# gkaissis/PriMIA

Measured on AMD Instinct MI355X. Metric: images_per_sec, higher is better.
Workload: dtype bf16; 1 GPU; ResNet-18 federated-client training step (fwd+loss+bwd+SGD), batch 256/client, 3x224x224, 1 client per GPU; batch_per_client=256, clients=1, sync_every_n_batch=3, dp_sgd=False

## Files before the change

### primia_amd/build.py

```python
import concurrent.futures
import os
import shutil
import subprocess
import sys

HERE = os.path.dirname(os.path.abspath(__file__))
CSRC = os.path.join(HERE, "csrc")
OBJ = os.path.join(CSRC, "_build")
ISA = os.path.join(OBJ, "isa")
LIB = os.path.join(HERE, "libprimia_hip.so")
ARCH = "gfx950"
FLAGS = ["-O3", "-std=c++17", "-fPIC", f"--offload-arch={ARCH}", "-Wno-unused-result"]


def source_digest(files=None):
    import hashlib

    names = sorted(f for f in os.listdir(CSRC) if f.endswith((".hip", ".h"))) if files is None else sorted(files)
    paths = [os.path.join(CSRC, f) for f in names]
    if files is None:
        paths.append(os.path.join(HERE, "..", "include", "primia_hip.h"))
    h = hashlib.sha256()
    for q in paths:
        h.update(os.path.basename(q).encode() + b"\0")
        import re

        text = re.sub(r"/\*.*?\*/", "", open(q, "r", encoding="utf-8", errors="replace").read(), flags=re.S)
        for line in text.splitlines():
            code = line.split("//", 1)[0].rstrip()
            if code:
                h.update(code.encode() + b"\n")
    return h.hexdigest()


def _hipcc():
    for c in ("/opt/rocm/bin/hipcc", "hipcc"):
        if os.path.isabs(c) and os.path.exists(c):
            return c
    return "hipcc"


def _newer(src, dst, deps=()):
    if not os.path.exists(dst):
        return True
    t = os.path.getmtime(dst)
    return any(os.path.getmtime(p) > t for p in (src, *deps))


def build(force=False, verbose=True):
    os.makedirs(OBJ, exist_ok=True)
    headers = [os.path.join(CSRC, f) for f in os.listdir(CSRC) if f.endswith(".h")]
    headers.append(os.path.join(HERE, "..", "include", "primia_hip.h"))
    sources = sorted(f for f in os.listdir(CSRC) if f.endswith(".hip"))
    jobs = []
    for f in sources:
        src = os.path.join(CSRC, f)
        obj = os.path.join(OBJ, f[:-4] + ".o")
        if force or _newer(src, obj, headers) or not os.path.exists(os.path.join(ISA, f[:-4] + ".s")):
            jobs.append((src, obj))

    def compile_one(job):
        src, obj = job
        name = os.path.basename(src)[:-4]
        tmp = os.path.join(OBJ, "tmp_" + name)
        shutil.rmtree(tmp, ignore_errors=True)
        os.makedirs(tmp)
        cmd = [_hipcc(), *FLAGS, "-save-temps=obj", "-c", src, "-o", os.path.join(tmp, name + ".o")]
        r = subprocess.run(cmd, capture_output=True, text=True)
        if r.returncode == 0:
            os.makedirs(ISA, exist_ok=True)
            os.replace(os.path.join(tmp, f"{name}-hip-amdgcn-amd-amdhsa-{ARCH}.s"), os.path.join(ISA, name + ".s"))
            os.replace(os.path.join(tmp, name + ".o"), obj)
        shutil.rmtree(tmp, ignore_errors=True)
        return src, r.returncode, r.stdout + r.stderr

    if jobs:
        with concurrent.futures.ThreadPoolExecutor(max_workers=min(6, len(jobs))) as ex:
            for src, rc, out in ex.map(compile_one, jobs):
                if verbose:
                    print(f"[primia build] {os.path.basename(src)}: {'ok' if rc == 0 else 'FAILED'}")
                if rc != 0:
                    raise RuntimeError(f"hipcc failed for {src}:\n{out}")
    objs = [os.path.join(OBJ, f[:-4] + ".o") for f in sources]
    if jobs or force or not os.path.exists(LIB):
        cmd = [_hipcc(), "-shared", "-fPIC", f"--offload-arch={ARCH}", "-o", LIB, *objs]
        r = subprocess.run(cmd, capture_output=True, text=True)
        if r.returncode != 0:
            raise RuntimeError("link failed:\n" + r.stdout + r.stderr)
        if verbose:
            print(f"[primia build] linked {LIB}")
    return LIB


PROBE_LIB = os.path.join(HERE, "..", "tools", "micro", "libprimia_probe.so")
PROBE_SOURCES = ("conv3x3_c64.hip", "conv_s2lh.hip", "options.hip")


def build_probe(extra_flags=()):
    build(verbose=False)
    objs = []
    for f in sorted(x for x in os.listdir(CSRC) if x.endswith(".hip")):
        if f in PROBE_SOURCES:
            os.makedirs(os.path.join(OBJ, "probe"), exist_ok=True)
            obj = os.path.join(OBJ, "probe", f[:-4] + ".o")
            cmd = [_hipcc(), *FLAGS, "-DPRIMIA_PROBE=1", *extra_flags, "-c", os.path.join(CSRC, f), "-o", obj]
            r = subprocess.run(cmd, capture_output=True, text=True)
            if r.returncode != 0:
                raise RuntimeError(f"hipcc failed for {f} (probe):\n{r.stdout}{r.stderr}")
        else:
            obj = os.path.join(OBJ, f[:-4] + ".o")
        objs.append(obj)
    r = subprocess.run([_hipcc(), "-shared", "-fPIC", f"--offload-arch={ARCH}", "-o", PROBE_LIB, *objs],
                       capture_output=True, text=True)
    if r.returncode != 0:
        raise RuntimeError("link failed:\n" + r.stdout + r.stderr)
    print(f"[primia build] linked {os.path.normpath(PROBE_LIB)}")
    return PROBE_LIB


if __name__ == "__main__":
    if "--probe" in sys.argv:
        build_probe()
    else:
        build(force="--force" in sys.argv)
```

### primia_amd/csrc/options.h

```cpp
#pragma once

namespace primia {

#define PRIMIA_OPTIONS(X)                                                                                              \
    X(lh2, 1)                                        \
    X(lh2_bm, 0)                                      \
    X(lh4, 1)                \
    X(c64_blocks, 512)                                         \
    X(c64_dbg, 0)                      \
    X(c64_stages, 4)                                                      \
    X(s2lh, 1)               \
    X(s2lh_dbg, 0)

enum OptId : int {
#define PRIMIA_OPT_ENUM(name, def) kOpt_##name,
    PRIMIA_OPTIONS(PRIMIA_OPT_ENUM)
#undef PRIMIA_OPT_ENUM
        kOptCount
};

extern int g_options[kOptCount];

inline int opt(OptId id) { return __atomic_load_n(&g_options[id], __ATOMIC_RELAXED); }

}

#define PRIMIA_OPT(name) (::primia::opt(::primia::kOpt_##name))
```

### primia_amd/csrc/options.hip

```cpp
#include <string.h>

#include <atomic>

#include "common.h"
#include "options.h"

#ifndef PRIMIA_PROBE
#define PRIMIA_PROBE 0
#endif

namespace primia {

int g_options[kOptCount] = {
#define PRIMIA_OPT_DEF(name, def) def,
    PRIMIA_OPTIONS(PRIMIA_OPT_DEF)
#undef PRIMIA_OPT_DEF
};

static const char* const kOptNames[kOptCount] = {
#define PRIMIA_OPT_NAME(name, def) #name,
    PRIMIA_OPTIONS(PRIMIA_OPT_NAME)
#undef PRIMIA_OPT_NAME
};

static const int kOptDefaults[kOptCount] = {
#define PRIMIA_OPT_DEF(name, def) def,
    PRIMIA_OPTIONS(PRIMIA_OPT_DEF)
#undef PRIMIA_OPT_DEF
};

static std::atomic<int64_t> g_options_epoch{0};

static int find_option(const char* name) {
    if (!name) return -1;
    for (int i = 0; i < kOptCount; ++i)
        if (!strcmp(name, kOptNames[i])) return i;
    return -1;
}

}

using namespace primia;

extern "C" {

int primia_set_option(const char* name, int value) {
    const int i = find_option(name);
    if (i < 0) return PRIMIA_ERR_ARG;
#if !PRIMIA_PROBE
    if ((i == kOpt_c64_dbg || i == kOpt_s2lh_dbg) && value != 0) return PRIMIA_ERR_UNSUPPORTED;
#endif
    if (__atomic_exchange_n(&g_options[i], value, __ATOMIC_RELAXED) != value)
        g_options_epoch.fetch_add(1, std::memory_order_release);
    return PRIMIA_OK;
}

int64_t primia_options_epoch(void) { return g_options_epoch.load(std::memory_order_acquire); }

int primia_get_option(const char* name, int* value) {
    const int i = find_option(name);
    if (i < 0 || !value) return PRIMIA_ERR_ARG;
    *value = __atomic_load_n(&g_options[i], __ATOMIC_RELAXED);
    return PRIMIA_OK;
}

int primia_reset_options(void) {
    bool moved = false;
    for (int i = 0; i < kOptCount; ++i) moved |= __atomic_exchange_n(&g_options[i], kOptDefaults[i], __ATOMIC_RELAXED) != kOptDefaults[i];
    if (moved) g_options_epoch.fetch_add(1, std::memory_order_release);
    return PRIMIA_OK;
}

int primia_option_count(void) { return kOptCount; }

int primia_option_name(int index, char* buf, int buf_len) {
    if (index < 0 || index >= kOptCount || !buf || buf_len <= (int)strlen(kOptNames[index])) return PRIMIA_ERR_ARG;
    strcpy(buf, kOptNames[index]);
    return PRIMIA_OK;
}

}
```

### primia_amd/csrc/stem_bwd_fused.hip

```cpp
#include <stdlib.h>

#include "conv_wgrad.h"

namespace primia {

__device__ __attribute__((aligned(16))) const unsigned char kStemFusedZeroPage[16] = {0};

__device__ __forceinline__ void sbf_dma16(const void* g, unsigned lds_addr) {
    asm volatile("s_mov_b32 m0, %1\n\ts_nop 0\n\tglobal_load_lds_dwordx4 %0, off" ::"v"(g), "s"(lds_addr) : "memory");
}

typedef int sbf_i32x4 __attribute__((ext_vector_type(4)));

__device__ __forceinline__ void sbf_bdma16(unsigned voff, sbf_i32x4 rsrc, unsigned lds_addr) {
    asm volatile("s_mov_b32 m0, %2\n\ts_nop 0\n\tbuffer_load_dwordx4 %0, %1, 0 offen lds"
                 ::"v"(voff), "s"(rsrc), "s"(lds_addr) : "memory");
}

__device__ __forceinline__ sbf_i32x4 sbf_rsrc(const void* base, long bytes) {
    const unsigned long long a = (unsigned long long)base;
    sbf_i32x4 r;
    r[0] = (int)(unsigned)a;
    r[1] = (int)(unsigned)(a >> 32) & 0xffff;
    r[2] = (int)(unsigned)(bytes > 0xfffffff0L ? 0xfffffff0L : bytes);
    r[3] = 0x00020000;
#pragma unroll
    for (int j = 0; j < 4; ++j) r[j] = __builtin_amdgcn_readfirstlane(r[j]);
    return r;
}
constexpr unsigned kSbfOob = 0xfffffff0u;

__device__ __forceinline__ int sbf_key(int slot) { return ((slot >> 1) & 1) | (((slot >> 3) & 1) << 1); }

__device__ __forceinline__ void sbf_wait_vmcnt(int n) {
    switch (n) {
        case 0: asm volatile("s_waitcnt vmcnt(0)" ::: "memory"); break;
        case 1: asm volatile("s_waitcnt vmcnt(1)" ::: "memory"); break;
        case 2: asm volatile("s_waitcnt vmcnt(2)" ::: "memory"); break;
        case 3: asm volatile("s_waitcnt vmcnt(3)" ::: "memory"); break;
        case 4: asm volatile("s_waitcnt vmcnt(4)" ::: "memory"); break;
        case 5: asm volatile("s_waitcnt vmcnt(5)" ::: "memory"); break;
        case 6: asm volatile("s_waitcnt vmcnt(6)" ::: "memory"); break;
        case 7: asm volatile("s_waitcnt vmcnt(7)" ::: "memory"); break;
        default: asm volatile("s_waitcnt vmcnt(8)" ::: "memory"); break;
    }
}

struct StemFusedParams {
    const bf16* xp;
    const bf16* y;
    const bf16* dpool;
    const uint8_t* argmax;
    const float *gamma, *beta, *mean, *invstd, *dbeta, *dgamma;
    float inv_m;
    float* dw;
    float* ws;
    int N, Hp, Wp, Ho, Wo, Hq, Wq;
    int PH, PW, PPI;
    int total, per_block;
    int debug;
};

constexpr int kSbfXB = 7 * 1024;
constexpr int kSbfTile = 16 * 1024;
constexpr int kSbfRaw = kSbfTile + 9 * 1024;
constexpr int kSbfRing = 5;
constexpr int kSbfRaw0 = 3 * kSbfXB;
constexpr int kSbfLds = kSbfRaw0 + kSbfRing * kSbfRaw;

__global__ __launch_bounds__(1024) void stem_bwd_fused_kernel(StemFusedParams p) {
    typedef __attribute__((address_space(3))) bf16x4_t* lds4_t;
    extern __shared__ __attribute__((aligned(16))) char smem[];
    const int tid = threadIdx.x, lane = tid & 63;
    const int wave = __builtin_amdgcn_readfirstlane(tid >> 6);
    const unsigned lds0 = (unsigned)(size_t)(__attribute__((address_space(3))) char*)smem;

    const int t0 = blockIdx.x * p.per_block;
    int t1 = t0 + p.per_block;
    if (t1 > p.total) t1 = p.total;
    const int n = t1 - t0;
    if (n <= 0) return;
    int cn = t0 / p.PPI, cph, cpw;
    {
        const int rem = t0 - cn * p.PPI;
        cph = rem / p.PW;
        cpw = rem - cph * p.PW;
    }
    auto advance = [&](int& an, int& aph, int& apw) {
        if (++apw == p.PW) {
            apw = 0;
            if (++aph == p.PH) {
                aph = 0;
                ++an;
            }
        }
    };

    if (wave >= 8) {
        const int tw = wave - 8;
        const int npc = tw == 0 ? 4 : 3;
        const sbf_i32x4 rs_y = sbf_rsrc(p.y, (long)p.N * p.Ho * p.Wo * 128);
        const sbf_i32x4 rs_g = sbf_rsrc(p.dpool, (long)p.N * p.Hq * p.Wq * 128);
        const sbf_i32x4 rs_c = sbf_rsrc(p.argmax, (long)p.N * p.Hq * p.Wq * 64);
        unsigned prel[4];
        int prow[4], pcol[4];
#pragma unroll
        for (int it = 0; it < 4; ++it) {
            const int idx = tw + 8 * it;
            prow[it] = pcol[it] = 0;
            if (idx < 16) {
                const int slot = idx * 8 + (lane >> 3), sl = lane & 7;
                const int chunk = ((((sl >> 1) ^ sbf_key(slot)) << 1) | (sl & 1));
                prel[it] = (unsigned)((((slot >> 4) * p.Wo + (slot & 15)) * 64 + chunk * 8) * 2);
            } else {
                const bool grad = idx < 22;
                const int G = (grad ? idx - 16 : idx - 22) * 64 + lane;
                const int slot = grad ? G >> 3 : G >> 2, sub = grad ? G & 7 : G & 3;
                const int row = slot / 9, col = slot - 9 * row;
                prow[it] = slot < 45 ? row : 1 << 20;
                pcol[it] = col;
                prel[it] = (unsigned)(grad ? (row * p.Wq + col) * 128 + sub * 16 : (row * p.Wq + col) * 64 + sub * 16);
            }
        }
        auto stage_raw = [&](int rbuf) {
            const unsigned ybase = (unsigned)(((cn * p.Ho + cph * 8) * p.Wo + cpw * 16) * 128);
            const int A0 = cph * 4, B0 = cpw * 8;
            const unsigned wpix = (unsigned)((cn * p.Hq + A0) * p.Wq + B0);
            const int rmax = p.Hq - A0, cmax = p.Wq - B0;
            advance(cn, cph, cpw);
#pragma unroll
            for (int it = 0; it < 4; ++it) {
                const int idx = tw + 8 * it;
                if (idx >= 25) break;
                const unsigned dst = __builtin_amdgcn_readfirstlane(lds0 + kSbfRaw0 + rbuf * kSbfRaw + idx * 1024);
                if (idx < 16) {
                    sbf_bdma16(prel[it] + ybase, rs_y, dst);
                } else {
                    const bool ok = prow[it] < rmax && pcol[it] < cmax;
                    if (idx < 22)
                        sbf_bdma16(ok ? prel[it] + wpix * 128u : kSbfOob, rs_g, dst);
                    else
                        sbf_bdma16(ok ? prel[it] + wpix * 64u : kSbfOob, rs_c, dst);
                }
            }
        };
        const int tt = tid - 512;
        const int c8 = tt & 7, bcol = (tt >> 3) & 7, brow = tw & 3, dg = tw >> 2;
        float k0[8], k1[8], k2[8], k3[8], k4[8], k5[8];
#pragma unroll
        for (int k = 0; k < 8; ++k) {
            const int c = c8 * 8 + k;
            const float is = p.invstd[c];
            k0[k] = p.mean[c];
            k1[k] = is;
            k2[k] = p.gamma[c] * is;
            k3[k] = p.dbeta[c] * p.inv_m;
            k4[k] = p.dgamma[c] * p.inv_m;
            k5[k] = p.beta[c];
        }
        __builtin_amdgcn_s_waitcnt(0x0f70);
        int tph = cph, tpw = cpw;
        typedef __attribute__((address_space(3))) char* ldsp_t;
        int offy[2];
#pragma unroll
        for (int r = 0; r < 2; ++r) {
            const int slot = (2 * brow + r) * 16 + 2 * bcol + (r ^ dg);
            offy[r] = slot * 128 + ((((c8 >> 1) ^ sbf_key(slot)) << 5) | ((c8 & 1) << 4));
        }
        const int offg = kSbfTile + (brow * 9 + bcol) * 128 + c8 * 16;
        const int offc = kSbfTile + 6 * 1024 + (brow * 9 + bcol) * 64 + c8 * 8;
        auto transform = [&](int rbuf) {
            const ldsp_t tile = (ldsp_t)(size_t)(lds0 + kSbfRaw0 + rbuf * kSbfRaw);
            const ldsp_t wg = tile + offg, wc = tile + offc;
            const bool rok = tph * 4 + brow + 1 < p.Hq, cok = tpw * 8 + bcol + 1 < p.Wq;
            if (++tpw == p.PW) {
                tpw = 0;
                if (++tph == p.PH) tph = 0;
            }
#pragma unroll
            for (int r = 0; r < 2; ++r) {
                const int j = r ^ dg;
                const ldsp_t yp = tile + offy[r];
                float vy[8], g[8];
                const u32x4 yraw = *(const __attribute__((address_space(3))) u32x4*)yp;
                Chunk<bf16>::unpack(yraw, vy);
#pragma unroll
                for (int k = 0; k < 8; ++k) g[k] = 0.f;
#pragma unroll
                for (int di = 1; di >= 0; --di) {
                    if (di > r) continue;
#pragma unroll
                    for (int dj = 1; dj >= 0; --dj) {
                        if (dj > j) continue;
                        const unsigned want = (unsigned)((1 + r - 2 * di) * 3 + (1 + j - 2 * dj));
                        const bool ok = (di == 0 || rok) && (dj == 0 || cok);
                        float wv[8];
                        const u32x4 wraw = *(const __attribute__((address_space(3))) u32x4*)(wg + (di * 9 + dj) * 128);
                        Chunk<bf16>::unpack(wraw, wv);
                        u32x2 codes = *(const __attribute__((address_space(3))) u32x2*)(wc + (di * 9 + dj) * 64);
                        if (!ok) codes = u32x2{0xffffffffu, 0xffffffffu};
#pragma unroll
                        for (int k = 0; k < 8; ++k)
                            g[k] += ((codes[k >> 2] >> (8 * (k & 3))) & 0xffu) == want ? wv[k] : 0.f;
                    }
                }
#pragma unroll
                for (int k = 0; k < 8; ++k) {
                    const float zz = __builtin_fmaf(vy[k] - k0[k], k2[k], k5[k]);
                    const float gi = zz > 0.f ? g[k] : 0.f;
                    const float xh = (vy[k] - k0[k]) * k1[k];
                    vy[k] = k2[k] * (gi - k3[k] - xh * k4[k]);
                }
                *(__attribute__((address_space(3))) u32x4*)yp = Chunk<bf16>::pack(vy);
            }
        };

        const bool raw_on = !(p.debug & 4);
        for (int s = 0; s < 3; ++s)
            if (s < n && raw_on) stage_raw(s);
        for (int k = -1; k < n; ++k) {
            const int inflight = (k + 2 < n ? npc : 0) + (k + 3 < n ? npc : 0);
            sbf_wait_vmcnt(raw_on ? inflight : 0);
            asm volatile("s_waitcnt lgkmcnt(0)" ::: "memory");
            __builtin_amdgcn_s_barrier();
            if (k + 4 < n && raw_on) stage_raw((k + 4) % kSbfRing);
            if (k + 1 < n && !(p.debug & 1)) transform((k + 1) % kSbfRing);
        }
        return;
    }

    const int kh = wave >> 2, rq = wave & 3;
    const int fr = lane & 15, fg = lane >> 4;
    const int tp = fr >> 2, tc8 = (fr & 3) * 8;
    const sbf_i32x4 rs_x = sbf_rsrc(p.xp, (long)p.N * p.Hp * p.Wp * 8);
    unsigned xrel;
    {
        const int G = wave * 64 + lane;
        const int row = G / 20, c16 = G - row * 20;
        xrel = G < 420 ? (unsigned)((row * p.Wp + 2 * c16) * 8) : kSbfOob;
    }
    auto stage_x = [&](int buf) {
        const unsigned xbase = (unsigned)(((cn * p.Hp + cph * 16) * p.Wp + cpw * 32) * 8);
        advance(cn, cph, cpw);
        if (wave < 7)
            sbf_bdma16(xrel == kSbfOob ? kSbfOob : xrel + xbase, rs_x,
                       __builtin_amdgcn_readfirstlane(lds0 + buf * kSbfXB + wave * 1024));
    };

    f32x4 acc[2][2][2];
#pragma unroll
    for (int i = 0; i < 2; ++i)
#pragma unroll
        for (int rr = 0; rr < 2; ++rr)
#pragma unroll
            for (int h = 0; h < 2; ++h) acc[i][rr][h] = f32x4{0.f, 0.f, 0.f, 0.f};

    typedef __attribute__((address_space(3))) char* ldsp_t;
    const int a_slot = 8 * fg + tp;
    int offa[2][2];
#pragma unroll
    for (int i = 0; i < 2; ++i)
#pragma unroll
        for (int h = 0; h < 2; ++h) {
            const int s0 = a_slot + 4 * h;
            offa[i][h] = s0 * 128 + (((2 * kh + i) ^ sbf_key(s0)) << 5) + tc8;
        }
    const int offb = ((fg >> 1) * 2) * 320 + 16 * (8 * (fg & 1) + tp) + tc8 + 2 * rq * 320;

    auto compute = [&](int xbuf, int rbuf) {
        const ldsp_t lb = (ldsp_t)(size_t)(lds0 + xbuf * kSbfXB) + offb;
        const ldsp_t la = (ldsp_t)(size_t)(lds0 + kSbfRaw0 + rbuf * kSbfRaw);
        ldsp_t pa[2][2];
#pragma unroll
        for (int i = 0; i < 2; ++i)
#pragma unroll
            for (int h = 0; h < 2; ++h) pa[i][h] = la + offa[i][h];
#pragma unroll
        for (int ks = 0; ks < 4; ++ks) {
            bf16x8_t a[2], b[2][2];
#pragma unroll
            for (int i = 0; i < 2; ++i) {
                bf16x4_t lo = __builtin_amdgcn_ds_read_tr16_b64_v4bf16((lds4_t)(pa[i][0] + ks * 4096));
                bf16x4_t hi = __builtin_amdgcn_ds_read_tr16_b64_v4bf16((lds4_t)(pa[i][1] + ks * 4096));
                a[i] = __builtin_shufflevector(lo, hi, 0, 1, 2, 3, 4, 5, 6, 7);
            }
#pragma unroll
            for (int rr = 0; rr < 2; ++rr) {
#pragma unroll
                for (int h = 0; h < 2; ++h) {
                    const ldsp_t q = lb + ((4 * ks + rr) * 320 + 32 * h);
                    bf16x4_t lo = __builtin_amdgcn_ds_read_tr16_b64_v4bf16((lds4_t)q);
                    bf16x4_t hi = __builtin_amdgcn_ds_read_tr16_b64_v4bf16((lds4_t)(q + 64));
                    b[rr][h] = __builtin_shufflevector(lo, hi, 0, 1, 2, 3, 4, 5, 6, 7);
                }
            }
#pragma unroll
            for (int rr = 0; rr < 2; ++rr) {
                if (2 * rq + rr == 7) continue;
#pragma unroll
                for (int h = 0; h < 2; ++h)
#pragma unroll
                    for (int i = 0; i < 2; ++i)
                        acc[i][rr][h] = __builtin_amdgcn_mfma_f32_16x16x32_bf16(a[i], b[rr][h], acc[i][rr][h], 0, 0, 0);
            }
        }
    };

    stage_x(0);
    if (n > 1) stage_x(1);
    for (int k = -1; k < n; ++k) {
        if (k + 1 < n && wave < 7)
            asm volatile("s_waitcnt vmcnt(1)" ::: "memory");
        else
            asm volatile("s_waitcnt vmcnt(0)" ::: "memory");
        __builtin_amdgcn_s_barrier();
        if (k < 0) continue;
        if (k + 2 < n) stage_x((k + 2) % 3);
        if (!(p.debug & 2)) compute(k % 3, k % kSbfRing);
    }

    if (p.ws) {
        float* o = p.ws + (long)blockIdx.x * (64 * 256);
#pragma unroll
        for (int rr = 0; rr < 2; ++rr) {
            const int r = 2 * rq + rr;
#pragma unroll
            for (int h = 0; h < 2; ++h) {
                const bool live = r < 7 && 16 * h + fr < 28;
#pragma unroll
                for (int i = 0; i < 2; ++i)
#pragma unroll
                    for (int j = 0; j < 4; ++j)
                        o[(32 * kh + 16 * i + 4 * fg + j) * 256 + r * 32 + 16 * h + fr] = live ? acc[i][rr][h][j] : 0.f;
            }
        }
        return;
    }
#pragma unroll
    for (int rr = 0; rr < 2; ++rr) {
        const int r = 2 * rq + rr;
        if (r == 7) continue;
#pragma unroll
        for (int h = 0; h < 2; ++h) {
            if (16 * h + fr >= 28) continue;
#pragma unroll
            for (int i = 0; i < 2; ++i)
#pragma unroll
                for (int j = 0; j < 4; ++j)
                    unsafeAtomicAdd(p.dw + (long)(32 * kh + 16 * i + 4 * fg + j) * 256 + r * 32 + 16 * h + fr, acc[i][rr][h][j]);
        }
    }
}

}

using namespace primia;

extern "C" int primia_stem_bwd_fused_ok(int N, int H, int W, int dtype) {
    if (dtype != PRIMIA_BF16 || N <= 0 || H <= 0 || W <= 0 || H % 32 != 0 || W % 32 != 0) return 0;
    if ((long)N * (H + 6) * (W + 8) * 4 >= (1L << 31) || (long)N * (H / 2) * (W / 2) * 64 >= (1L << 31)) return 0;
    int total, per_block, grid;
    return stem_wgrad_halo_blocks(N, H, W, &total, &per_block, &grid) ? 1 : 0;
}

extern "C" int primia_stem_bwd_fused(const void* x_padded, const void* y, const void* dpooled, const uint8_t* argmax,
                                     const float* gamma, const float* beta, const float* save_mean,
                                     const float* save_invstd, const float* dgamma, const float* dbeta, float* dw_acc,
                                     void* ws, int64_t ws_bytes, int N, int H, int W, int dtype,
                                     primia_stream_t stream) {
    PRIMIA_REQUIRE(x_padded && y && dpooled && argmax && gamma && beta && save_mean && save_invstd && dgamma && dbeta &&
                   dw_acc && N > 0 && H > 0 && W > 0);
    if (dtype != PRIMIA_BF16) return PRIMIA_ERR_UNSUPPORTED;
    if (H % 32 != 0 || W % 32 != 0) return PRIMIA_ERR_UNSUPPORTED;
    if ((long)N * (H + 6) * (W + 8) * 4 >= (1L << 31) || (long)N * (H / 2) * (W / 2) * 64 >= (1L << 31))
        return PRIMIA_ERR_UNSUPPORTED;
    StemFusedParams p;
    p.xp = (const bf16*)x_padded; p.y = (const bf16*)y; p.dpool = (const bf16*)dpooled; p.argmax = argmax;
    p.gamma = gamma; p.beta = beta; p.mean = save_mean; p.invstd = save_invstd; p.dbeta = dbeta; p.dgamma = dgamma;
    p.dw = dw_acc;
    p.N = N; p.Hp = H + 6; p.Wp = W + 8; p.Ho = H / 2; p.Wo = W / 2;
    p.Hq = (p.Ho + 2 - 3) / 2 + 1; p.Wq = (p.Wo + 2 - 3) / 2 + 1;
    p.inv_m = (float)(1.0 / ((double)N * p.Ho * p.Wo));
    p.PH = p.Ho / 8; p.PW = p.Wo / 16; p.PPI = p.PH * p.PW;
    int grid = 0;
    if (!stem_wgrad_halo_blocks(N, H, W, &p.total, &p.per_block, &grid)) return PRIMIA_ERR_UNSUPPORTED;
    const int64_t slab_bytes = (int64_t)grid * 64 * 256 * (int64_t)sizeof(float);
    const bool store = ws && ws_bytes >= slab_bytes;
    p.ws = store ? (float*)ws : nullptr;
    p.debug = 0;
    static bool attr_set = false;
    if (!attr_set) {
        if (hipFuncSetAttribute((const void*)stem_bwd_fused_kernel, hipFuncAttributeMaxDynamicSharedMemorySize, kSbfLds) !=
            hipSuccess)
            return PRIMIA_ERR_LAUNCH;
        attr_set = true;
    }
    hipStream_t st = (hipStream_t)stream;
    stem_bwd_fused_kernel<<<grid, 1024, kSbfLds, st>>>(p);
    if (store) wgrad_tile_reduce(p.ws, dw_acc, grid, 1, 64, 256, 1, 1, 4, 256, 1, st);
    return launch_status();
}
```

Before: 55100 images/s.

## Move stem-bwd raw tile loads from transform waves to MFMA waves

Moves the async buffer loads of the raw y/dpool/argmax tiles off the transform waves and onto the compute (MFMA) waves, interleaving them with the x-tile staging in one vmcnt-tracked pipeline. Transform waves get raised scheduling priority so their elementwise work is not starved. Compute is reordered to run before issuing the next stage loads, with a sched_barrier in between. Debug bits are gated behind a probe build option. The rebalancing adds load-issue and wait pressure to the compute waves, and the wait accounting is more complex.

```diff
diff --git a/primia_amd/build.py b/primia_amd/build.py
--- a/primia_amd/build.py
+++ b/primia_amd/build.py
@@ -93,7 +93,7 @@
 
 
 PROBE_LIB = os.path.join(HERE, "..", "tools", "micro", "libprimia_probe.so")
-PROBE_SOURCES = ("conv3x3_c64.hip", "conv_s2lh.hip", "options.hip")
+PROBE_SOURCES = ("conv3x3_c64.hip", "conv_s2lh.hip", "stem_bwd_fused.hip", "options.hip")
 
 
 def build_probe(extra_flags=()):
diff --git a/primia_amd/csrc/options.h b/primia_amd/csrc/options.h
--- a/primia_amd/csrc/options.h
+++ b/primia_amd/csrc/options.h
@@ -10,7 +10,8 @@
     X(c64_dbg, 0)                      \
     X(c64_stages, 4)                                                      \
     X(s2lh, 1)               \
-    X(s2lh_dbg, 0)
+    X(s2lh_dbg, 0)           \
+    X(stem_bwd_dbg, 0)
 
 enum OptId : int {
 #define PRIMIA_OPT_ENUM(name, def) kOpt_##name,
diff --git a/primia_amd/csrc/options.hip b/primia_amd/csrc/options.hip
--- a/primia_amd/csrc/options.hip
+++ b/primia_amd/csrc/options.hip
@@ -48,7 +48,7 @@
     const int i = find_option(name);
     if (i < 0) return PRIMIA_ERR_ARG;
 #if !PRIMIA_PROBE
-    if ((i == kOpt_c64_dbg || i == kOpt_s2lh_dbg) && value != 0) return PRIMIA_ERR_UNSUPPORTED;
+    if ((i == kOpt_c64_dbg || i == kOpt_s2lh_dbg || i == kOpt_stem_bwd_dbg) && value != 0) return PRIMIA_ERR_UNSUPPORTED;
 #endif
     if (__atomic_exchange_n(&g_options[i], value, __ATOMIC_RELAXED) != value)
         g_options_epoch.fetch_add(1, std::memory_order_release);
diff --git a/primia_amd/csrc/stem_bwd_fused.hip b/primia_amd/csrc/stem_bwd_fused.hip
--- a/primia_amd/csrc/stem_bwd_fused.hip
+++ b/primia_amd/csrc/stem_bwd_fused.hip
@@ -1,6 +1,7 @@
 #include <stdlib.h>
 
 #include "conv_wgrad.h"
+#include "options.h"
 
 namespace primia {
 
@@ -45,6 +46,11 @@
         default: asm volatile("s_waitcnt vmcnt(8)" ::: "memory"); break;
     }
 }
+
+#ifndef PRIMIA_PROBE
+#define PRIMIA_PROBE 0
+#endif
+#define SBF_DBG(bit) (PRIMIA_PROBE && (p.debug & (bit)))
 
 struct StemFusedParams {
     const bf16* xp;
@@ -98,52 +104,7 @@
 
     if (wave >= 8) {
         const int tw = wave - 8;
-        const int npc = tw == 0 ? 4 : 3;
-        const sbf_i32x4 rs_y = sbf_rsrc(p.y, (long)p.N * p.Ho * p.Wo * 128);
-        const sbf_i32x4 rs_g = sbf_rsrc(p.dpool, (long)p.N * p.Hq * p.Wq * 128);
-        const sbf_i32x4 rs_c = sbf_rsrc(p.argmax, (long)p.N * p.Hq * p.Wq * 64);
-        unsigned prel[4];
-        int prow[4], pcol[4];
-#pragma unroll
-        for (int it = 0; it < 4; ++it) {
-            const int idx = tw + 8 * it;
-            prow[it] = pcol[it] = 0;
-            if (idx < 16) {
-                const int slot = idx * 8 + (lane >> 3), sl = lane & 7;
-                const int chunk = ((((sl >> 1) ^ sbf_key(slot)) << 1) | (sl & 1));
-                prel[it] = (unsigned)((((slot >> 4) * p.Wo + (slot & 15)) * 64 + chunk * 8) * 2);
-            } else {
-                const bool grad = idx < 22;
-                const int G = (grad ? idx - 16 : idx - 22) * 64 + lane;
-                const int slot = grad ? G >> 3 : G >> 2, sub = grad ? G & 7 : G & 3;
-                const int row = slot / 9, col = slot - 9 * row;
-                prow[it] = slot < 45 ? row : 1 << 20;
-                pcol[it] = col;
-                prel[it] = (unsigned)(grad ? (row * p.Wq + col) * 128 + sub * 16 : (row * p.Wq + col) * 64 + sub * 16);
-            }
-        }
-        auto stage_raw = [&](int rbuf) {
-            const unsigned ybase = (unsigned)(((cn * p.Ho + cph * 8) * p.Wo + cpw * 16) * 128);
-            const int A0 = cph * 4, B0 = cpw * 8;
-            const unsigned wpix = (unsigned)((cn * p.Hq + A0) * p.Wq + B0);
-            const int rmax = p.Hq - A0, cmax = p.Wq - B0;
-            advance(cn, cph, cpw);
-#pragma unroll
-            for (int it = 0; it < 4; ++it) {
-                const int idx = tw + 8 * it;
-                if (idx >= 25) break;
-                const unsigned dst = __builtin_amdgcn_readfirstlane(lds0 + kSbfRaw0 + rbuf * kSbfRaw + idx * 1024);
-                if (idx < 16) {
-                    sbf_bdma16(prel[it] + ybase, rs_y, dst);
-                } else {
-                    const bool ok = prow[it] < rmax && pcol[it] < cmax;
-                    if (idx < 22)
-                        sbf_bdma16(ok ? prel[it] + wpix * 128u : kSbfOob, rs_g, dst);
-                    else
-                        sbf_bdma16(ok ? prel[it] + wpix * 64u : kSbfOob, rs_c, dst);
-                }
-            }
-        };
+        if (!SBF_DBG(16)) __builtin_amdgcn_s_setprio(3);
         const int tt = tid - 512;
         const int c8 = tt & 7, bcol = (tt >> 3) & 7, brow = tw & 3, dg = tw >> 2;
         float k0[8], k1[8], k2[8], k3[8], k4[8], k5[8];
@@ -215,19 +176,60 @@
             }
         };
 
-        const bool raw_on = !(p.debug & 4);
-        for (int s = 0; s < 3; ++s)
-            if (s < n && raw_on) stage_raw(s);
         for (int k = -1; k < n; ++k) {
-            const int inflight = (k + 2 < n ? npc : 0) + (k + 3 < n ? npc : 0);
-            sbf_wait_vmcnt(raw_on ? inflight : 0);
             asm volatile("s_waitcnt lgkmcnt(0)" ::: "memory");
             __builtin_amdgcn_s_barrier();
-            if (k + 4 < n && raw_on) stage_raw((k + 4) % kSbfRing);
-            if (k + 1 < n && !(p.debug & 1)) transform((k + 1) % kSbfRing);
+            if (k + 1 < n && !SBF_DBG(1)) transform((k + 1) % kSbfRing);
         }
         return;
     }
+
+    const int npc = wave == 7 ? 4 : 3;
+    const sbf_i32x4 rs_y = sbf_rsrc(p.y, (long)p.N * p.Ho * p.Wo * 128);
+    const sbf_i32x4 rs_g = sbf_rsrc(p.dpool, (long)p.N * p.Hq * p.Wq * 128);
+    const sbf_i32x4 rs_c = sbf_rsrc(p.argmax, (long)p.N * p.Hq * p.Wq * 64);
+    unsigned prel[4];
+    int prow[2], pcol[2];
+#pragma unroll
+    for (int it = 0; it < 4; ++it) {
+        const int idx = it < 3 ? wave + 8 * it : 24;
+        if (it < 2) {
+            const int slot = idx * 8 + (lane >> 3), sl = lane & 7;
+            const int chunk = ((((sl >> 1) ^ sbf_key(slot)) << 1) | (sl & 1));
+            prel[it] = (unsigned)((((slot >> 4) * p.Wo + (slot & 15)) * 64 + chunk * 8) * 2);
+        } else {
+            const bool grad = idx < 22;
+            const int G = (grad ? idx - 16 : idx - 22) * 64 + lane;
+            const int slot = grad ? G >> 3 : G >> 2, sub = grad ? G & 7 : G & 3;
+            const int row = slot / 9, col = slot - 9 * row;
+            prow[it - 2] = slot < 45 ? row : 1 << 20;
+            pcol[it - 2] = col;
+            prel[it] = (unsigned)(grad ? (row * p.Wq + col) * 128 + sub * 16 : (row * p.Wq + col) * 64 + sub * 16);
+        }
+    }
+    int rn = cn, rph = cph, rpw = cpw;
+    auto stage_raw = [&](int rbuf) {
+        const unsigned ybase = (unsigned)(((rn * p.Ho + rph * 8) * p.Wo + rpw * 16) * 128);
+        const int A0 = rph * 4, B0 = rpw * 8;
+        const unsigned wpix = (unsigned)((rn * p.Hq + A0) * p.Wq + B0);
+        const int rmax = p.Hq - A0, cmax = p.Wq - B0;
+        advance(rn, rph, rpw);
+#pragma unroll
+        for (int it = 0; it < 4; ++it) {
+            if (it == 3 && wave != 7) break;
+            const int idx = it < 3 ? wave + 8 * it : 24;
+            const unsigned dst = __builtin_amdgcn_readfirstlane(lds0 + kSbfRaw0 + rbuf * kSbfRaw + idx * 1024);
+            if (it < 2) {
+                sbf_bdma16(prel[it] + ybase, rs_y, dst);
+            } else {
+                const bool ok = prow[it - 2] < rmax && pcol[it - 2] < cmax;
+                if (idx < 22)
+                    sbf_bdma16(ok ? prel[it] + wpix * 128u : kSbfOob, rs_g, dst);
+                else
+                    sbf_bdma16(ok ? prel[it] + wpix * 64u : kSbfOob, rs_c, dst);
+            }
+        }
+    };
 
     const int kh = wave >> 2, rq = wave & 3;
     const int fr = lane & 15, fg = lane >> 4;
@@ -306,17 +308,25 @@
         }
     };
 
+    const bool raw_on = !SBF_DBG(4);
+    const int nraw = raw_on ? npc : 0, npx = wave < 7 ? 1 : 0;
     stage_x(0);
-    if (n > 1) stage_x(1);
+    for (int s = 0; s < 3; ++s)
+        if (s < n && raw_on) stage_raw(s);
     for (int k = -1; k < n; ++k) {
-        if (k + 1 < n && wave < 7)
-            asm volatile("s_waitcnt vmcnt(1)" ::: "memory");
-        else
-            asm volatile("s_waitcnt vmcnt(0)" ::: "memory");
+        sbf_wait_vmcnt((k + 2 < n ? nraw : 0) + (k >= 0 && k + 1 < n ? npx : 0) + (k + 3 < n ? nraw : 0));
         __builtin_amdgcn_s_barrier();
-        if (k < 0) continue;
+        if (SBF_DBG(8)) {
+            if (k + 2 < n) stage_x((k + 2) % 3);
+            if (k + 4 < n && raw_on) stage_raw((k + 4) % kSbfRing);
+            __builtin_amdgcn_sched_barrier(0);
+            if (k >= 0 && !SBF_DBG(2)) compute(k % 3, k % kSbfRing);
+            continue;
+        }
+        if (k >= 0 && !SBF_DBG(2)) compute(k % 3, k % kSbfRing);
+        __builtin_amdgcn_sched_barrier(0);
         if (k + 2 < n) stage_x((k + 2) % 3);
-        if (!(p.debug & 2)) compute(k % 3, k % kSbfRing);
+        if (k + 4 < n && raw_on) stage_raw((k + 4) % kSbfRing);
     }
 
     if (p.ws) {
@@ -387,7 +397,7 @@
     const int64_t slab_bytes = (int64_t)grid * 64 * 256 * (int64_t)sizeof(float);
     const bool store = ws && ws_bytes >= slab_bytes;
     p.ws = store ? (float*)ws : nullptr;
-    p.debug = 0;
+    p.debug = PRIMIA_PROBE ? PRIMIA_OPT(stem_bwd_dbg) : 0;
     static bool attr_set = false;
     if (!attr_set) {
         if (hipFuncSetAttribute((const void*)stem_bwd_fused_kernel, hipFuncAttributeMaxDynamicSharedMemorySize, kSbfLds) !=
```

Result: no change. 54970 images/s (-0.2%).
